# flupkede/codesearch

Hardware: AMD Instinct MI355X
Metric: chunks embedded+searched/sec over 10M×384 corpus; recall@10 vs CPU ref (higher is better)
Workload: dtype f32

## Files before the change

codesearch_amd/csrc/attention_split.hip:

```cpp
#include <cstdlib>
#include "encoder.hpp"
#include "split_f16.hpp"
#include "attention_shx_body.hpp"

#ifndef AT_STAMP
#define AT_STAMP(i)
#endif

namespace cs {

#ifndef CS_ATTN_PIPE_WAVES
#define CS_ATTN_PIPE_WAVES 3
#endif

constexpr int kAttnPipeDefault32 = 2, kAttnPipeDefault64 = 3;

#ifdef CS_DIAGNOSTICS
__global__ void __launch_bounds__(256, 2)
attention_sh2_kernel(const _Float16* __restrict__ qkvs, const int32_t* __restrict__ mask,
                     _Float16* __restrict__ ctxs, uint32_t* __restrict__ flag, uint32_t L, uint32_t H,
                     float scale_log2e) {
    extern __shared__ __attribute__((aligned(16))) char smem[];
    const uint32_t Lp = (L + 31) & ~31u;
    char* Kt = smem;
    char* Vt = Kt + (size_t)Lp * 128;
    float* madd = reinterpret_cast<float*>(Vt + (size_t)Lp * 128);
    int* last_valid_p = reinterpret_cast<int*>(madd + Lp);
    const int tid = threadIdx.x, lane = tid & 63;
    const int wave = __builtin_amdgcn_readfirstlane(tid >> 6);
    const int l31 = lane & 31, h = lane >> 5;
    const uint32_t head = blockIdx.x, b = blockIdx.y;
    const uint32_t nh = H / 32, nch = 3 * nh;
    const _Float16* base = qkvs + (size_t)b * L * nch * 64;
    bool ovf = false;

    AT_STAMP(0);
    if (tid == 0) *last_valid_p = 0;
    for (uint32_t ii = wave; ii < Lp / 8; ii += 4) {
        const uint32_t row = ii * 8 + (lane >> 3);
        const uint32_t key = row < L ? row : L - 1;
        const uint32_t ck = (lane & 7) ^ ((row >> 1) & 7);
        const uint32_t cv = (lane & 7) ^ (4 * ((row >> 1) & 1));
        sh_glds16(base + ((size_t)key * nch + nh + head) * 64 + ck * 8, Kt + ii * 1024);
        sh_glds16(base + ((size_t)key * nch + 2 * nh + head) * 64 + cv * 8, Vt + ii * 1024);
    }
    __syncthreads();
    for (uint32_t key = tid; key < Lp; key += 256) {
        const bool ok = key < L && mask[(size_t)b * L + key] != 0;
// ... 93 lines not shown
                oxx = __builtin_amdgcn_mfma_f32_32x32x16_f16(vh.v, pl[s].v, oxx, 0, 0, 0);
                oxx = __builtin_amdgcn_mfma_f32_32x32x16_f16(vl.v, ph[s].v, oxx, 0, 0, 0);
            }
        }
        lsum += __shfl_xor(lsum, 32, 64);
        const float inv = 1.0f / lsum;
        if (query < L) {
            _Float16* op = ctxs + (((size_t)b * L + query) * nh + head) * 64 + 4 * h;
#pragma unroll
            for (int g = 0; g < 4; ++g) {
                f16x4 hi, lo;
#pragma unroll
                for (int e = 0; e < 4; ++e) {
                    _Float16 a, bb;
                    ovf |= sh_split(fmaf(oxx[4 * g + e], kShLoInv, ohh[4 * g + e]) * inv, a, bb);
                    hi[e] = a; lo[e] = bb;
                }
                *reinterpret_cast<f16x4*>(op + 8 * g) = hi;
                *reinterpret_cast<f16x4*>(op + 32 + 8 * g) = lo;
            }
        }
    }
    AT_STAMP(2);
    if (ovf && flag) atomicOr(flag, 1u);
}
#endif

template <int NC, int POS = 0, int PIPE = 0>
__global__ void __launch_bounds__(256, NC == 1 ? (PIPE == 1 ? CS_ATTN_PIPE_WAVES : (PIPE >= 2 ? 4 : 2)) : 2)
attention_shx_kernel(const _Float16* __restrict__ qkvs, const int32_t* __restrict__ mask,
                     _Float16* __restrict__ ctxs, uint32_t* __restrict__ flag, uint32_t L, uint32_t H,
                     float scale_log2e, uint32_t HB, float* __restrict__ range_out,
                     const uint32_t* __restrict__ seq_unit, const uint32_t* __restrict__ unit_len,
                     const float* __restrict__ alibi_log2, uint32_t window) {
    extern __shared__ __attribute__((aligned(16))) char smem[];
    const AttnMemPlain mem;
    attention_shx_body<NC, AttnMemPlain, AttnMemPlain, POS, PIPE>(smem, mem, mem, qkvs, mask, ctxs, flag, L, H, scale_log2e, HB, range_out,
                                                            seq_unit, unit_len, blockIdx.x, blockIdx.y, blockIdx.z, gridDim.x,
                                                            gridDim.z, alibi_log2, window);
}

namespace {

struct ShxArgs {
    const _Float16* qkv; const int32_t* mask; _Float16* ctx; uint32_t* flag; uint32_t L, H; float scale_log2e; uint32_t hb;
    float* range_out; const uint32_t* seq_unit; const uint32_t* unit_len; const float* alibi_log2; uint32_t window;
};

template <int NC, int POS, int PIPE>
int32_t launch_shx_one(dim3 grid, size_t lds, hipStream_t s, const ShxArgs& a) {
    if (lds > 64 * 1024 - 256) {
        static PerDeviceOnce attr;
        CS_TRY(attr.run([&]() -> int32_t {
            CS_HIP(hipFuncSetAttribute(reinterpret_cast<const void*>(attention_shx_kernel<NC, POS, PIPE>),
                                       hipFuncAttributeMaxDynamicSharedMemorySize, 160 * 1024 - 64));
            return CS_OK;
        }));
    }
    hipLaunchKernelGGL((attention_shx_kernel<NC, POS, PIPE>), grid, dim3(256), lds, s, a.qkv, a.mask, a.ctx, a.flag, a.L, a.H,
                       a.scale_log2e, a.hb, a.range_out, a.seq_unit, a.unit_len, a.alibi_log2, a.window);
    CS_HIP(hipGetLastError());
    return CS_OK;
}

template <int NC>
int32_t launch_shx(int pos, int pipe, dim3 grid, size_t lds, hipStream_t s, const ShxArgs& a) {
#ifndef CS_DIAGNOSTICS
    constexpr int P = NC == 1 ? kAttnPipeDefault32 : kAttnPipeDefault64;
    (void)pipe;
    if (pos == 1) return launch_shx_one<NC, 1, P>(grid, lds, s, a);
    if (pos == 2) return launch_shx_one<NC, 2, P>(grid, lds, s, a);
    return launch_shx_one<NC, 0, P>(grid, lds, s, a);
#else
    if (pipe == 3) {
        if (pos == 1) return launch_shx_one<NC, 1, 3>(grid, lds, s, a);
        if (pos == 2) return launch_shx_one<NC, 2, 3>(grid, lds, s, a);
        return launch_shx_one<NC, 0, 3>(grid, lds, s, a);
    }
    if (pipe == 2) {
        if (pos == 1) return launch_shx_one<NC, 1, 2>(grid, lds, s, a);
        if (pos == 2) return launch_shx_one<NC, 2, 2>(grid, lds, s, a);
        return launch_shx_one<NC, 0, 2>(grid, lds, s, a);
    }
    if (pipe == 1) {
        if (pos == 1) return launch_shx_one<NC, 1, 1>(grid, lds, s, a);
        if (pos == 2) return launch_shx_one<NC, 2, 1>(grid, lds, s, a);
        return launch_shx_one<NC, 0, 1>(grid, lds, s, a);
    }
    if (pos == 1) return launch_shx_one<NC, 1, 0>(grid, lds, s, a);
    if (pos == 2) return launch_shx_one<NC, 2, 0>(grid, lds, s, a);
    return launch_shx_one<NC, 0, 0>(grid, lds, s, a);
#endif
}

}

int32_t launch_attention_sh2(const _Float16* qkv_split, const int32_t* mask, void* ctx_split, uint32_t* flag,
                             uint32_t B, uint32_t L, uint32_t H, uint32_t heads, hipStream_t s, float* range_out,
                             uint32_t* range_pairs, const uint32_t* seq_unit, const uint32_t* unit_len, const float* alibi,
                             uint32_t window) {
    if (alibi && window) return fail(CS_ERR_BAD_ARG, "attention: ALiBi and a local window together are not built");
    const float* alibi_log2 = alibi ? alibi + heads : nullptr;
    const int pos = alibi_log2 ? 1 : (window ? 2 : 0);
    if (range_pairs) *range_pairs = 0;
    const uint32_t dh = heads ? H / heads : 0;
    if ((dh != 32 && dh != 64) || H % heads)
        return fail(CS_ERR_UNSUPPORTED, "head_dim %u not supported (32 or 64)", dh);
    const size_t Lp = (L + 31) & ~31u;
    static const int pipe_env = [] { const char* e = cs_lab_env("CS_ATTN_PIPE"); return e && e[0] >= '0' && e[0] <= '3' ? e[0] - '0' : -1; }();
    ShxArgs a{qkv_split, mask, static_cast<_Float16*>(ctx_split), flag, L, H, 0.0f, 1u, range_out, seq_unit, unit_len, alibi_log2, window};
    if (dh == 64) {
        const size_t lds = 2 * 2 * 128 * 128 + Lp * sizeof(float) + 16;
        a.scale_log2e = (1.0f / sqrtf(64.0f)) * kLog2e;
        const int pipe = pipe_env < 0 ? kAttnPipeDefault64 : pipe_env;
        CS_TRY(launch_shx<2>(pos, pipe, dim3(heads, B, (L + 127) / 128), lds, s, a));
        if (range_pairs) *range_pairs = heads * B * ((L + 127) / 128) * 4;
        return CS_OK;
    }
    static const bool shx1 = [] { const char* e = cs_lab_env("CS_ATTN_SHX1"); return !(e && e[0] == '0'); }();
    if (shx1 || pos) {
        static const size_t lds_pad = [] { const char* e = cs_lab_env("CS_ATTN_LDS_PAD"); return e ? (size_t)std::atol(e) : (size_t)0; }();
        const size_t lds1 = 2 * 1 * 128 * 128 + Lp * sizeof(float) + 16 + lds_pad;
        static const bool pack_heads = [] { const char* e = cs_lab_env("CS_ATTN_PACK_HEADS"); return !(e && e[0] == '0'); }();
        uint32_t hb = !pack_heads ? 1u : (Lp <= 32 ? 4u : (Lp <= 64 ? 2u : 1u));
        while (heads % hb) hb >>= 1;
        a.scale_log2e = (1.0f / sqrtf(32.0f)) * kLog2e;
        a.hb = hb;
        const int pipe = pipe_env < 0 ? kAttnPipeDefault32 : pipe_env;
        CS_TRY(launch_shx<1>(pos, pipe, dim3(heads / hb, B, (L + 127) / 128), lds1, s, a));
        if (range_pairs) *range_pairs = (heads / hb) * B * ((L + 127) / 128) * 4;
        return CS_OK;
    }
#ifndef CS_DIAGNOSTICS
    return fail(CS_ERR_UNSUPPORTED, "attention: no kernel for head_dim %u", dh);
#else
    const size_t lds = 2 * Lp * 128 + Lp * sizeof(float) + 16;
    if (lds > 160 * 1024 - 64) return fail(CS_ERR_UNSUPPORTED, "sequence length %u exceeds the LDS-resident K/V limit", L);
    static PerDeviceOnce attr_set;
    CS_TRY(attr_set.run([&]() -> int32_t {
        CS_HIP(hipFuncSetAttribute(reinterpret_cast<const void*>(attention_sh2_kernel),
                                   hipFuncAttributeMaxDynamicSharedMemorySize, 160 * 1024 - 64));
        return CS_OK;
// ... 10 lines not shown
```

codesearch_amd/csrc/attention_shx_body.hpp:

```cpp
#pragma once

#include "encoder.hpp"
#include "split_f16.hpp"

#ifndef AT_STAMP
#define AT_STAMP(i)
#endif
#ifndef CS_ATTN_ARITH
#define CS_ATTN_ARITH 2
#endif
#ifndef CS_ATTN_LAZY_RESCALE
#define CS_ATTN_LAZY_RESCALE 4.0f
#endif
#ifndef CS_ATTN_PIPE_FENCE
#define CS_ATTN_PIPE_FENCE __builtin_amdgcn_sched_barrier(0)
#endif

namespace cs {

typedef __fp16 h16x2 __attribute__((ext_vector_type(2)));

constexpr float kLog2e = 1.4426950408889634f;
constexpr float kMaskedLog2 = -3.0e38f;

union Frag8 {
    f16x8 v;
    uint32_t u[4];
    uint2 d[2];
};

typedef short s16x4 __attribute__((ext_vector_type(4)));

union FragTr {
    f16x8 v;
    s16x4 q[2];
};

__device__ __forceinline__ void split_pair_rtz_ng(float a, float b, uint32_t& hi, uint32_t& lo) {
    const h16x2 h = __builtin_amdgcn_cvt_pkrtz(a, b);
    const h16x2 l = __builtin_amdgcn_cvt_pkrtz((a - (float)h[0]) * kShLoScale, (b - (float)h[1]) * kShLoScale);
    hi = __builtin_bit_cast(uint32_t, h);
    lo = __builtin_bit_cast(uint32_t, l);
}

__device__ __forceinline__ float mix_residual_lo(float e, uint32_t hpair) {
    float r;
    asm("v_fma_mix_f32 %0, %1, -1.0, %2 op_sel_hi:[1,0,0]" : "=v"(r) : "v"(hpair), "v"(e));
    return r;
}
__device__ __forceinline__ float mix_residual_hi(float e, uint32_t hpair) {
    float r;
    asm("v_fma_mix_f32 %0, %1, -1.0, %2 op_sel:[1,0,0] op_sel_hi:[1,0,0]" : "=v"(r) : "v"(hpair), "v"(e));
    return r;
}

__device__ __forceinline__ float xhalf_max_swap(float t) {
    const uint32_t u = __builtin_bit_cast(uint32_t, t);
    const auto r = __builtin_amdgcn_permlane32_swap(u, u, false, false);
    const uint32_t a = r[0], b = r[1];
    return fmaxf(__builtin_bit_cast(float, a), __builtin_bit_cast(float, b));
}

struct AttnMemPlain {
    __device__ __forceinline__ f16x8 ld16(const _Float16* p) const { return *reinterpret_cast<const f16x8*>(p); }
    __device__ __forceinline__ f16x8 stage_load(const _Float16* src, char* lds_piece) const { sh_glds16(src, lds_piece); return f16x8{}; }
    __device__ __forceinline__ void stage_store(char*, int, f16x8) const {}
    __device__ __forceinline__ void st8(_Float16* p, f16x4 v) const { *reinterpret_cast<f16x4*>(p) = v; }
};

template <int NC, class MQ, class MO, int POS = 0, int PIPE = 0>
__device__ __forceinline__ void
attention_shx_body(char* smem, const MQ& mq, const MO& mo, const _Float16* qkvs, const int32_t* __restrict__ mask,
                   _Float16* ctxs, uint32_t* __restrict__ flag, uint32_t L, uint32_t H,
                   float scale_log2e, uint32_t HB, float* __restrict__ range_out,
                   const uint32_t* __restrict__ seq_unit, const uint32_t* __restrict__ unit_len,
                   uint32_t bx, uint32_t by, uint32_t bz, uint32_t gx, uint32_t gz, const float* __restrict__ alibi_log2 = nullptr,
                   uint32_t window = 0) {
    constexpr bool ALIBI = POS == 1, WINDOW = POS == 2;
    constexpr bool IMM = PIPE >= 2;
    constexpr bool EARLY = PIPE == 3;
    const float wlimit = (float)window;
    constexpr int KT = 128;
    const uint32_t Lp = (L + 31) & ~31u;
    char* Kt = smem;
    char* Vt = Kt + (size_t)NC * KT * 128;
    float* madd = reinterpret_cast<float*>(Vt + (size_t)NC * KT * 128);
    int* last_valid_p = reinterpret_cast<int*>(madd + Lp);
    const int tid = threadIdx.x, lane = tid & 63;
    const int wave = __builtin_amdgcn_readfirstlane(tid >> 6);
    const int l31 = lane & 31, h = lane >> 5;
    const uint32_t wq = 4 / HB, hsub = (uint32_t)wave / wq, qt = (uint32_t)wave % wq;
    const uint32_t head = bx * HB + hsub, b = by, qb = bz;
    Kt += (size_t)hsub * (KT / HB) * 128;
    Vt += (size_t)hsub * (KT / HB) * 128;
    const uint32_t nh = H / (32 * NC), nch = 3 * nh * NC;
    const _Float16* base = qkvs + (size_t)b * L * nch * 64;
    bool ovf = false;

    AT_STAMP(0);
    if (tid == 0) *last_valid_p = 0;

    const int kswz = (l31 >> 1) & 7;
    int k_hi[2], k_lo[2];
#pragma unroll
    for (int s = 0; s < 2; ++s) {
        k_hi[s] = ((2 * s + h) ^ kswz) * 16;
        k_lo[s] = ((4 + 2 * s + h) ^ kswz) * 16;
    }
    const int vq = (lane & 15) >> 2, vp = lane & 3, vg = (lane >> 4) & 1;
    const int vfv = 4 * ((vq >> 1) & 1);
    const int v_hi = (4 * h + vq) * 128 + (((2 * vg + (vp >> 1)) ^ vfv) * 16) + 8 * (vp & 1);
    const int v_lo = v_hi ^ 64;

    const bool wave_live = qb * 128 + qt * 32 < L;
    const uint32_t query = qb * 128 + qt * 32 + l31;
    const uint32_t qsrc = query < L ? query : L - 1;
    float neg_slope = 0.0f;
    const float qpos = (float)query - (float)(4 * h);
    if constexpr (ALIBI) neg_slope = -alibi_log2[head];
    f16x8 qh[NC][2], ql[NC][2];
#pragma unroll
    for (int c = 0; c < NC; ++c) {
        const _Float16* qp = base + ((size_t)qsrc * nch + head * NC + c) * 64 + 8 * h;
#pragma unroll
        for (int s = 0; s < 2; ++s) {
            qh[c][s] = mq.ld16(qp + 16 * s);
            ql[c][s] = mq.ld16(qp + 32 + 16 * s);
        }
    }
#if CS_ATTN_ARITH == 2 && !defined(CS_ATTN_SCALAR_SOFTMAX)
    f16x8 qhs[NC][2];
#pragma unroll
    for (int c = 0; c < NC; ++c)
#pragma unroll
        for (int s = 0; s < 2; ++s) {
            qhs[c][s] = qh[c][s] * (_Float16)kShLoInv;
            ql[c][s] = ql[c][s] * (_Float16)kShLoInv;
        }
#endif
    sh_f32x16 ohh[NC], oxx[NC];
#pragma unroll
    for (int c = 0; c < NC; ++c)
#pragma unroll
        for (int r = 0; r < 16; ++r) { ohh[c][r] = 0.0f; oxx[c][r] = 0.0f; }
    float m = -__builtin_huge_valf(), lsum = 0.0f;

    auto stage = [&](uint32_t st) {
        const uint32_t live = Lp - st * KT < (uint32_t)KT ? Lp - st * KT : (uint32_t)KT;
        for (uint32_t i0 = qt; i0 < live / 8; i0 += 4 * wq) {
            f16x8 rk[4][NC], rv[4][NC];
#pragma unroll
            for (int u = 0; u < 4; ++u) {
                const uint32_t ii = i0 + u * wq;
                if (ii < live / 8) {
                    const uint32_t row = ii * 8 + (lane >> 3);
                    const uint32_t gk = st * KT + row;
                    const uint32_t key = gk < L ? gk : L - 1;
                    const uint32_t ck = (lane & 7) ^ ((row >> 1) & 7);
                    const uint32_t cv = (lane & 7) ^ (4 * ((row >> 1) & 1));
#pragma unroll
                    for (int c = 0; c < NC; ++c) {
                        rk[u][c] = mq.stage_load(base + ((size_t)key * nch + (nh + head) * NC + c) * 64 + ck * 8, Kt + (size_t)c * KT * 128 + ii * 1024);
                        rv[u][c] = mq.stage_load(base + ((size_t)key * nch + (2 * nh + head) * NC + c) * 64 + cv * 8, Vt + (size_t)c * KT * 128 + ii * 1024);
                    }
                }
            }
#pragma unroll
            for (int u = 0; u < 4; ++u) {
                const uint32_t ii = i0 + u * wq;
                if (ii < live / 8) {
#pragma unroll
                    for (int c = 0; c < NC; ++c) {
                        mq.stage_store(Kt + (size_t)c * KT * 128 + ii * 1024, lane, rk[u][c]);
                        mq.stage_store(Vt + (size_t)c * KT * 128 + ii * 1024, lane, rv[u][c]);
                    }
                }
            }
        }
    };
    stage(0);
    __syncthreads();
    for (uint32_t key = tid; key < Lp; key += 256) {
        const bool ok = key < L && mask[(size_t)b * L + key] != 0;
        madd[key] = ok ? 0.0f : kMaskedLog2;
        if (ok) atomicMax(last_valid_p, (int)key);
    }
    asm volatile("s_waitcnt vmcnt(0)" ::: "memory");
    __syncthreads();
    const uint32_t ntiles = (uint32_t)(*last_valid_p) / 32 + 1;

    typedef __attribute__((address_space(3))) char* lds_char_p;
    typedef __attribute__((address_space(3))) const f16x8* lds_f16x8_cp;
    typedef __attribute__((address_space(3))) const sh_f32x4* lds_f32x4_cp;
    uint32_t ka[4] = {0, 0, 0, 0}, va[2] = {0, 0}, ma0 = 0;
    if constexpr (IMM) {
        const uint32_t k0 = (uint32_t)(uintptr_t)(lds_char_p)Kt + (uint32_t)l31 * 128u, v0 = (uint32_t)(uintptr_t)(lds_char_p)Vt;
#pragma unroll
        for (int s = 0; s < 2; ++s) { ka[s] = k0 + (uint32_t)k_hi[s]; ka[2 + s] = k0 + (uint32_t)k_lo[s]; }
        va[0] = v0 + (uint32_t)v_hi;
        va[1] = v0 + (uint32_t)v_lo;
        ma0 = (uint32_t)(uintptr_t)(lds_char_p)reinterpret_cast<char*>(madd) + 16u * (uint32_t)h;
#pragma unroll
        for (int i = 0; i < 4; ++i) asm volatile("" : "+v"(ka[i]));
        asm volatile("" : "+v"(va[0]), "+v"(va[1]), "+v"(ma0));
    }

    for (uint32_t st = 0; st * 4 < ntiles; ++st) {
        if constexpr (WINDOW) {
            if (st * KT > qb * 128 + 127 + window || st * KT + (KT - 1) + window < qb * 128) continue;
        }
        if (st > 0) {
            __syncthreads();
            stage(st);
            asm volatile("s_waitcnt vmcnt(0)" ::: "memory");
            __syncthreads();
        }
        if (!wave_live) continue;
        const uint32_t kt_end = ntiles - st * 4 < 4 ? ntiles - st * 4 : 4;
        const uint32_t ma_st = ma0 + st * 512u;
        uint32_t kl_lo = 0, kl_hi = kt_end;
        if constexpr (WINDOW) {
            const int q0 = (int)(qb * 128 + qt * 32), w = (int)window, t0 = (int)(st * 4);
            const int first = q0 - 31 - w > 0 ? (q0 - 31 - w + 31) / 32 : 0, past = (q0 + 31 + w) / 32 + 1;
            kl_lo = (uint32_t)(first > t0 ? first - t0 : 0);
            kl_hi = past - t0 < (int)kt_end ? (uint32_t)(past - t0 > 0 ? past - t0 : 0) : kt_end;
        }
        auto compute_s = [&](uint32_t kl, sh_f32x16& hh, sh_f32x16& xx) __attribute__((always_inline)) {
#pragma unroll
            for (int r = 0; r < 16; ++r) { hh[r] = 0.0f; xx[r] = 0.0f; }
            if constexpr (EARLY) {
                f16x8 kf[NC][4];
#pragma unroll
                for (int c = 0; c < NC; ++c)
#pragma unroll
                    for (int i = 0; i < 4; ++i) kf[c][i] = *(lds_f16x8_cp)(uintptr_t)(ka[i] + (uint32_t)(c * KT * 128) + kl * 4096u);
                __builtin_amdgcn_sched_barrier(0);
#pragma unroll
                for (int c = 0; c < NC; ++c)
#pragma unroll
                    for (int s = 0; s < 2; ++s) {
                        hh = __builtin_amdgcn_mfma_f32_32x32x16_f16(kf[c][s], qh[c][s], hh, 0, 0, 0);
#if CS_ATTN_ARITH == 2 && !defined(CS_ATTN_SCALAR_SOFTMAX)
                        hh = __builtin_amdgcn_mfma_f32_32x32x16_f16(kf[c][s], ql[c][s], hh, 0, 0, 0);
                        hh = __builtin_amdgcn_mfma_f32_32x32x16_f16(kf[c][2 + s], qhs[c][s], hh, 0, 0, 0);
#else
                        xx = __builtin_amdgcn_mfma_f32_32x32x16_f16(kf[c][s], ql[c][s], xx, 0, 0, 0);
                        xx = __builtin_amdgcn_mfma_f32_32x32x16_f16(kf[c][2 + s], qh[c][s], xx, 0, 0, 0);
#endif
                    }
                return;
            }
#pragma unroll
            for (int c = 0; c < NC; ++c) {
                const char* kr = Kt + (size_t)c * KT * 128 + (size_t)(kl * 32 + l31) * 128;
#pragma unroll
                for (int s = 0; s < 2; ++s) {
                    f16x8 kh, kl8;
                    if constexpr (IMM) {
                        kh = *(lds_f16x8_cp)(uintptr_t)(ka[s] + (uint32_t)(c * KT * 128) + kl * 4096u);
                        kl8 = *(lds_f16x8_cp)(uintptr_t)(ka[2 + s] + (uint32_t)(c * KT * 128) + kl * 4096u);
                    } else {
                        kh = *reinterpret_cast<const f16x8*>(kr + k_hi[s]);
                        kl8 = *reinterpret_cast<const f16x8*>(kr + k_lo[s]);
                    }
                    hh = __builtin_amdgcn_mfma_f32_32x32x16_f16(kh, qh[c][s], hh, 0, 0, 0);
#if CS_ATTN_ARITH == 2 && !defined(CS_ATTN_SCALAR_SOFTMAX)
                    hh = __builtin_amdgcn_mfma_f32_32x32x16_f16(kh, ql[c][s], hh, 0, 0, 0);
                    hh = __builtin_amdgcn_mfma_f32_32x32x16_f16(kl8, qhs[c][s], hh, 0, 0, 0);
#else
                    xx = __builtin_amdgcn_mfma_f32_32x32x16_f16(kh, ql[c][s], xx, 0, 0, 0);
                    xx = __builtin_amdgcn_mfma_f32_32x32x16_f16(kl8, qh[c][s], xx, 0, 0, 0);
#endif
                }
            }
        };
        auto finish_tile = [&](uint32_t kl, sh_f32x16& hh, sh_f32x16& xx) __attribute__((always_inline)) {
            const uint32_t kt = st * 4 + kl;
#ifndef CS_ATTN_SCALAR_SOFTMAX
            sh_f32x2 p2[8];
            float tmax = -__builtin_huge_valf();
            const sh_f32x2 lo_inv2 = {kShLoInv, kShLoInv}, scale2 = {scale_log2e, scale_log2e};
#pragma unroll
            for (int g = 0; g < 4; ++g) {
                sh_f32x4 ma;
                if constexpr (IMM) ma = *(lds_f32x4_cp)(uintptr_t)(ma_st + (kl * 32u + 8u * g) * 4u);
                else ma = *reinterpret_cast<const sh_f32x4*>(madd + kt * 32 + 8 * g + 4 * h);
#pragma unroll
                for (int e2 = 0; e2 < 2; ++e2) {
                    const int r = 4 * g + 2 * e2;
                    const sh_f32x2 x2 = {xx[r], xx[r + 1]}, h2 = {hh[r], hh[r + 1]};
                    sh_f32x2 m2 = {ma[2 * e2], ma[2 * e2 + 1]};
                    if constexpr (ALIBI) {
                        const float d0 = qpos - (float)(kt * 32 + 8 * g + 2 * e2);
                        m2[0] = fmaf(neg_slope, fabsf(d0), m2[0]);
                        m2[1] = fmaf(neg_slope, fabsf(d0 - 1.0f), m2[1]);
                    }
                    if constexpr (WINDOW) {
                        const float d0 = qpos - (float)(kt * 32 + 8 * g + 2 * e2);
                        m2[0] = fabsf(d0) > wlimit ? kMaskedLog2 : m2[0];
                        m2[1] = fabsf(d0 - 1.0f) > wlimit ? kMaskedLog2 : m2[1];
                    }
#if CS_ATTN_ARITH == 2
                    (void)x2; (void)lo_inv2;
                    const sh_f32x2 s2 = __builtin_elementwise_fma(h2, scale2, m2);
#else
                    const sh_f32x2 s2 = __builtin_elementwise_fma(__builtin_elementwise_fma(x2, lo_inv2, h2), scale2, m2);
#endif
                    p2[r / 2] = s2;
                    tmax = fmaxf(tmax, fmaxf(s2[0], s2[1]));
                }
            }
            if constexpr (IMM) tmax = xhalf_max_swap(tmax);
            else tmax = fmaxf(tmax, __shfl_xor(tmax, 32, 64));
#if CS_ATTN_ARITH == 2
            if (__any(tmax > m + CS_ATTN_LAZY_RESCALE)) {
#else
            if (__any(tmax > m)) {
#endif
                const float mnew = fmaxf(m, tmax);
                const float alpha = __builtin_amdgcn_exp2f(m - mnew);
                lsum *= alpha;
#pragma unroll
                for (int c = 0; c < NC; ++c)
#pragma unroll
                    for (int r = 0; r < 16; ++r) { ohh[c][r] *= alpha; oxx[c][r] *= alpha; }
                m = mnew;
            }
            typedef __attribute__((address_space(3))) s16x4* lds_s16x4_p;
            FragTr vhe[NC][2], vle[NC][2];
            if constexpr (EARLY) {
#pragma unroll
                for (int c = 0; c < NC; ++c)
#pragma unroll
                    for (int s = 0; s < 2; ++s) {
                        const uint32_t off = (uint32_t)(c * KT * 128) + kl * 4096u + (uint32_t)(s * 16 * 128);
                        vhe[c][s].q[0] = __builtin_amdgcn_ds_read_tr16_b64_v4i16((lds_s16x4_p)(uintptr_t)(va[0] + off));
                        vhe[c][s].q[1] = __builtin_amdgcn_ds_read_tr16_b64_v4i16((lds_s16x4_p)(uintptr_t)(va[0] + off + 1024u));
                        vle[c][s].q[0] = __builtin_amdgcn_ds_read_tr16_b64_v4i16((lds_s16x4_p)(uintptr_t)(va[1] + off));
                        vle[c][s].q[1] = __builtin_amdgcn_ds_read_tr16_b64_v4i16((lds_s16x4_p)(uintptr_t)(va[1] + off + 1024u));
                    }
                __builtin_amdgcn_sched_barrier(0);
            }
#if CS_ATTN_ARITH == 2
            const sh_f32x2 m2v = {m - 11.0f, m - 11.0f};
#else
            const sh_f32x2 m2v = {m, m};
#endif
            sh_f32x2 ps2 = {0.0f, 0.0f};
            Frag8 ph[2], pl[2];
            const sh_f32x2 lo_scale2 = {kShLoScale, kShLoScale};
#pragma unroll
            for (int i = 0; i < 8; ++i) {
                const sh_f32x2 d2 = p2[i] - m2v;
                const sh_f32x2 e2 = {__builtin_amdgcn_exp2f(d2[0]), __builtin_amdgcn_exp2f(d2[1])};
                ps2 += e2;
                const h16x2 hi = __builtin_amdgcn_cvt_pkrtz(e2[0], e2[1]);
#if CS_ATTN_ARITH == 2
                (void)lo_scale2;
                const uint32_t hib = __builtin_bit_cast(uint32_t, hi);
                const h16x2 lo = __builtin_amdgcn_cvt_pkrtz(mix_residual_lo(e2[0], hib), mix_residual_hi(e2[1], hib));
#else
                const sh_f32x2 back = {(float)hi[0], (float)hi[1]};
                const sh_f32x2 r2 = (e2 - back) * lo_scale2;
                const h16x2 lo = __builtin_amdgcn_cvt_pkrtz(r2[0], r2[1]);
#endif
                ph[i >> 2].u[i & 3] = __builtin_bit_cast(uint32_t, hi);
                pl[i >> 2].u[i & 3] = __builtin_bit_cast(uint32_t, lo);
            }
            lsum += ps2[0] + ps2[1];
#else
            float tmax = -__builtin_huge_valf();
#pragma unroll
            for (int g = 0; g < 4; ++g) {
                const sh_f32x4 ma = *reinterpret_cast<const sh_f32x4*>(madd + kt * 32 + 8 * g + 4 * h);
#pragma unroll
                for (int e = 0; e < 4; ++e) {
                    const int r = 4 * g + e;
                    float me = ma[e];
                    if constexpr (ALIBI) me = fmaf(neg_slope, fabsf(qpos - (float)(kt * 32 + 8 * g + e)), me);
                    if constexpr (WINDOW) me = fabsf(qpos - (float)(kt * 32 + 8 * g + e)) > wlimit ? kMaskedLog2 : me;
                    hh[r] = fmaf(fmaf(xx[r], kShLoInv, hh[r]), scale_log2e, me);
                    tmax = fmaxf(tmax, hh[r]);
                }
            }
            tmax = fmaxf(tmax, __shfl_xor(tmax, 32, 64));
            if (__any(tmax > m)) {
                const float mnew = fmaxf(m, tmax);
                const float alpha = __builtin_amdgcn_exp2f(m - mnew);
                lsum *= alpha;
#pragma unroll
                for (int c = 0; c < NC; ++c)
#pragma unroll
                    for (int r = 0; r < 16; ++r) { ohh[c][r] *= alpha; oxx[c][r] *= alpha; }
                m = mnew;
            }
            float psum = 0.0f;
#pragma unroll
            for (int r = 0; r < 16; ++r) {
                hh[r] = __builtin_amdgcn_exp2f(hh[r] - m);
                psum += hh[r];
            }
            lsum += psum;
            Frag8 ph[2], pl[2];
#pragma unroll
            for (int s = 0; s < 2; ++s)
#pragma unroll
                for (int w2 = 0; w2 < 4; ++w2) {
#ifdef CS_ATTN_P_HI_ONLY
                    const f16x2 pr = __builtin_convertvector(sh_f32x2{hh[8 * s + 2 * w2], hh[8 * s + 2 * w2 + 1]}, f16x2);
                    ph[s].u[w2] = __builtin_bit_cast(uint32_t, pr);
                    pl[s].u[w2] = 0u;
#else
                    split_pair_rtz_ng(hh[8 * s + 2 * w2], hh[8 * s + 2 * w2 + 1], ph[s].u[w2], pl[s].u[w2]);
#endif
                }
#endif
#ifdef CS_ATTN_SCALAR_SOFTMAX
            typedef __attribute__((address_space(3))) s16x4* lds_s16x4_p;
            FragTr vhe[NC][2], vle[NC][2];
#endif
#pragma unroll
            for (int c = 0; c < NC; ++c) {
                const char* vr = Vt + (size_t)c * KT * 128 + (size_t)kl * 32 * 128;
#pragma unroll
                for (int s = 0; s < 2; ++s) {
                    FragTr vh, vl;
                    if constexpr (EARLY) {
                        vh = vhe[c][s];
                        vl = vle[c][s];
                    } else if constexpr (IMM) {
                        const uint32_t off = (uint32_t)(c * KT * 128) + kl * 4096u + (uint32_t)(s * 16 * 128);
                        vh.q[0] = __builtin_amdgcn_ds_read_tr16_b64_v4i16((lds_s16x4_p)(uintptr_t)(va[0] + off));
                        vh.q[1] = __builtin_amdgcn_ds_read_tr16_b64_v4i16((lds_s16x4_p)(uintptr_t)(va[0] + off + 1024u));
                        vl.q[0] = __builtin_amdgcn_ds_read_tr16_b64_v4i16((lds_s16x4_p)(uintptr_t)(va[1] + off));
                        vl.q[1] = __builtin_amdgcn_ds_read_tr16_b64_v4i16((lds_s16x4_p)(uintptr_t)(va[1] + off + 1024u));
                    } else {
                    vh.q[0] = __builtin_amdgcn_ds_read_tr16_b64_v4i16((lds_s16x4_p)(vr + s * 16 * 128 + v_hi));
                    vh.q[1] = __builtin_amdgcn_ds_read_tr16_b64_v4i16((lds_s16x4_p)(vr + s * 16 * 128 + 8 * 128 + v_hi));
                    vl.q[0] = __builtin_amdgcn_ds_read_tr16_b64_v4i16((lds_s16x4_p)(vr + s * 16 * 128 + v_lo));
                    vl.q[1] = __builtin_amdgcn_ds_read_tr16_b64_v4i16((lds_s16x4_p)(vr + s * 16 * 128 + 8 * 128 + v_lo));
                    }
                    ohh[c] = __builtin_amdgcn_mfma_f32_32x32x16_f16(vh.v, ph[s].v, ohh[c], 0, 0, 0);
#if CS_ATTN_ARITH == 2 && !defined(CS_ATTN_SCALAR_SOFTMAX)
                    ohh[c] = __builtin_amdgcn_mfma_f32_32x32x16_f16(vh.v, pl[s].v, ohh[c], 0, 0, 0);
#elif !defined(CS_ATTN_P_HI_ONLY)
                    oxx[c] = __builtin_amdgcn_mfma_f32_32x32x16_f16(vh.v, pl[s].v, oxx[c], 0, 0, 0);
#endif
                    oxx[c] = __builtin_amdgcn_mfma_f32_32x32x16_f16(vl.v, ph[s].v, oxx[c], 0, 0, 0);
                }
            }
        };
        if constexpr (PIPE == 0) {
            for (uint32_t kl = kl_lo; kl < kl_hi; ++kl) {
                sh_f32x16 hh, xx;
                compute_s(kl, hh, xx);
                finish_tile(kl, hh, xx);
            }
        } else if constexpr (IMM) {
#pragma unroll
            for (uint32_t kl = 0; kl < 4; ++kl) {
                if (kl >= kl_lo && kl < kl_hi) {
                    sh_f32x16 hh, xx;
                    compute_s(kl, hh, xx);
                    finish_tile(kl, hh, xx);
                }
            }
        } else {
            sh_f32x16 hhA, xxA, hhB, xxB;
            if (kl_lo < kl_hi) compute_s(kl_lo, hhA, xxA);
            for (uint32_t kl = kl_lo; kl < kl_hi; kl += 2) {
                if (kl + 1 < kl_hi) compute_s(kl + 1, hhB, xxB);
                CS_ATTN_PIPE_FENCE;
                finish_tile(kl, hhA, xxA);
                if (kl + 1 < kl_hi) {
                    if (kl + 2 < kl_hi) compute_s(kl + 2, hhA, xxA);
                    CS_ATTN_PIPE_FENCE;
                    finish_tile(kl + 1, hhB, xxB);
                }
            }
        }
    }
    lsum += __shfl_xor(lsum, 32, 64);
    const float inv = lsum > 0.0f ? 1.0f / lsum : 0.0f;
    float rlo = 0.0f, rhi = 0.0f;
    if (wave_live && query < L) {
#pragma unroll
        for (int c = 0; c < NC; ++c) {
            _Float16* op = ctxs + (((size_t)b * L + query) * nh + head) * NC * 64 + c * 64 + 4 * h;
#pragma unroll
            for (int g = 0; g < 4; ++g) {
                f16x4 hi, lo;
#pragma unroll
                for (int e = 0; e < 4; ++e) {
                    _Float16 a, bb;
                    const float o = fmaf(oxx[c][4 * g + e], kShLoInv, ohh[c][4 * g + e]) * inv;
                    ovf |= sh_split(o, a, bb);
                    hi[e] = a; lo[e] = bb;
                    rlo = fminf(rlo, o);
                    rhi = fmaxf(rhi, o);
                }
                mo.st8(op + 8 * g, hi);
                mo.st8(op + 32 + 8 * g, lo);
            }
        }
    }
    AT_STAMP(2);
    if (ovf && flag) atomicOr(flag, 1u);
    if (range_out) {
        if (unit_len && query >= unit_len[seq_unit[b]]) rlo = rhi = 0.0f;
#pragma unroll
        for (int o = 32; o > 0; o >>= 1) {
            rlo = fminf(rlo, __shfl_xor(rlo, o, 64));
            rhi = fmaxf(rhi, __shfl_xor(rhi, o, 64));
        }
        if (lane == 0) {
            const size_t blk = ((size_t)by * gz + bz) * gx + bx;
            _Float16 a, bb;
            (void)sh_split(rlo, a, bb);
            range_out[(blk * 4 + wave) * 2] = fmaf((float)bb, kShLoInv, (float)a);
            (void)sh_split(rhi, a, bb);
            range_out[(blk * 4 + wave) * 2 + 1] = fmaf((float)bb, kShLoInv, (float)a);
        }
    }
}

}
```

codesearch_amd/csrc/small_forward.hip:

```cpp
#include "small_forward.hpp"

#include "attention_shx_body.hpp"
#include "encoder_rows.hpp"
#include "gemm_epilogue.hpp"
#include "split_f16.hpp"

#include <type_traits>

namespace cs {

namespace {

typedef unsigned int sf_u32x4 __attribute__((ext_vector_type(4)));
typedef unsigned int sf_u32x2 __attribute__((ext_vector_type(2)));

constexpr int SF_GRID = 96;
constexpr int SF_W_BYTES = 16 * 12 * 128;
constexpr int SF_AROW = 384 * 4 + 16;
constexpr int SF_AIMG = 16 * SF_AROW;
constexpr int SF_RED = 4 * 16 * 17 * 4;
constexpr int SF_ATT = 2 * 128 * 128 + 512 * 4 + 16;
constexpr int SF_OFF_AIMG = SF_W_BYTES, SF_OFF_RED = SF_W_BYTES + SF_AIMG, SF_OFF_ATT = SF_W_BYTES;
constexpr int SF_LDS = SF_W_BYTES + (SF_ATT > SF_AIMG + SF_RED ? SF_ATT : SF_AIMG + SF_RED);
constexpr int SC1 = 16;
// ... 238 lines not shown
    using E_RESID = std::integral_constant<int, SH_OUT_F32_RESID>;
    using E_PART = std::integral_constant<int, SH_OUT_PARTIAL>;

    constexpr uint32_t NT_QKV = 3 * H / 16, NT_H = H / 16, NT_I = I / 16;
    const float scale_log2e = (1.0f / sqrtf(32.0f)) * kLog2e;

    {
        const SfMap m(NT_QKV, blk);
        if (m.active) sf_w_prefetch(lds_w, a.layers[0].wqkv, m.nt, KC_H, 0, KC_H, wave, lane);
        asm volatile("s_waitcnt vmcnt(0)" ::: "memory");
        __syncthreads();
    }

    for (uint32_t l = 0; l < a.n_layers; ++l) {
        const SfLayer ly = a.layers[l];
        {
            const SfMap m(NT_QKV, blk);
            if (m.active) {
                const float* gw = l ? a.layers[l - 1].ln2_g : a.emb_g;
                const float* bw = l ? a.layers[l - 1].ln2_b : a.emb_b;
                const float* pb = l ? a.layers[l - 1].bdown : nullptr;
                for (uint32_t mt = m.mt0; mt < MT; mt += m.mt_step) {
                    ln_prologue(mt, gw, bw, l ? 1 : 2, pb, m.nt == 0, a.XA, bXA);
                    tile(E_SPLIT{}, true, nullptr, nullptr, 0, 0, mt, m.nt, ly.bqkv, &bQ, 3 * H, nullptr, a.QKVS, 0);
                }
            }
        }
        if (!barrier(ly.wo, NT_H, KC_H, 5 * l + 1)) return;
        {
            const uint32_t hgroups = a.heads / a.hb, qblocks = (a.L + 127) / 128;
            const uint32_t tasks = hgroups * a.B * qblocks;
            for (uint32_t t = blk; t < tasks; t += SF_GRID) {
                const uint32_t bx = t % hgroups, by = (t / hgroups) % a.B, bz = t / (hgroups * a.B);
                attention_shx_body<1>(lds + SF_OFF_ATT, bQ, bC, a.QKVS, a.mask, a.CTXS, a.flag, a.L, H, scale_log2e, a.hb, nullptr,
                                      nullptr, nullptr, bx, by, bz, hgroups, qblocks);
                __syncthreads();
            }
        }
        if (!barrier(nullptr, 0, 0, 5 * l + 2)) return;
        {
            const SfMap m(NT_H, blk);
            if (m.active)
                for (uint32_t mt = m.mt0; mt < MT; mt += m.mt_step)
                    tile(E_RESID{}, false, &bC, a.CTXS, KC_H, 0, mt, m.nt, ly.bo, &bY, H, a.Y, nullptr, 0);
        }
        if (!barrier(ly.wup, NT_I, KC_H, 5 * l + 3)) return;
        {
            const SfMap m(NT_I, blk);
            if (m.active)
                for (uint32_t mt = m.mt0; mt < MT; mt += m.mt_step) {
                    ln_prologue(mt, ly.ln1_g, ly.ln1_b, 0, nullptr, m.nt == 0, a.X, bX);
                    tile(E_GELU{}, true, nullptr, nullptr, 0, 0, mt, m.nt, ly.bup, &bM, I, nullptr, a.MIDS, 0);
                }
        }
        if (!barrier(ly.wdown, NT_H, KC_I, 5 * l + 4, true)) return;
        {
            const SfMap m(NT_H, blk);
            if (m.active)
                for (uint32_t mt = 0; mt < MT; ++mt)
                    tile(E_PART{}, false, &bM, a.MIDS, KC_I, m.mt0 * (KC_I / 4), mt, m.nt, nullptr, &bP, H, a.PARTS, nullptr, m.mt0);
        }
        const bool last = l + 1 == a.n_layers;
        if (!barrier(last ? nullptr : a.layers[l + 1].wqkv, NT_QKV, KC_H, 5 * l + 5)) return;
    }
    {
        const SfLayer ly = a.layers[a.n_layers - 1];
        for (uint32_t t = 4 * blk + wave; t < T; t += 4 * SF_GRID) {
// ... 45 lines not shown
```

Baseline: 4.625 billion.

## Remap attention blocks to a 1D grid so each XCD keeps one head group

Launches the attention kernel on a flattened 1D grid and remaps the linear block id so that all query blocks of a (batch, head) group land on the same XCD, assuming round-robin block dispatch across the eight XCDs. The goal is to keep a group's K/V reads inside one XCD's L2 instead of spreading them across all of them. This adds index arithmetic per block plus a check on the total block count, and the old grid order remains available only as a diagnostic fallback.

Result: no change. 4.621 billion (-0.1%).

```diff
diff --git a/codesearch_amd/csrc/attention_split.hip b/codesearch_amd/csrc/attention_split.hip
--- a/codesearch_amd/csrc/attention_split.hip
+++ b/codesearch_amd/csrc/attention_split.hip
@@ -2,6 +2,7 @@
 #include "encoder.hpp"
 #include "split_f16.hpp"
 #include "attention_shx_body.hpp"
+#include "attn_dispatch.hpp"
 
 #ifndef AT_STAMP
 #define AT_STAMP(i)
@@ -173,12 +174,20 @@
                      _Float16* __restrict__ ctxs, uint32_t* __restrict__ flag, uint32_t L, uint32_t H,
                      float scale_log2e, uint32_t HB, float* __restrict__ range_out,
                      const uint32_t* __restrict__ seq_unit, const uint32_t* __restrict__ unit_len,
-                     const float* __restrict__ alibi_log2, uint32_t window) {
+                     const float* __restrict__ alibi_log2, uint32_t window, uint32_t gx, uint32_t groups, uint32_t gz,
+                     uint32_t grid_order) {
     extern __shared__ __attribute__((aligned(16))) char smem[];
     const AttnMemPlain mem;
+    AttnBlock blk = attn_dispatch(blockIdx.x, groups, gz);
+#ifdef CS_DIAGNOSTICS
+    if (grid_order) blk = attn_dispatch_grid_order(blockIdx.x, groups);
+#else
+    (void)grid_order;
+#endif
+    const uint32_t group = __builtin_amdgcn_readfirstlane(blk.group), bz = __builtin_amdgcn_readfirstlane(blk.qb);
+    const uint32_t by = __builtin_amdgcn_readfirstlane(group / gx), bx = group - by * gx;
     attention_shx_body<NC, AttnMemPlain, AttnMemPlain, POS, PIPE>(smem, mem, mem, qkvs, mask, ctxs, flag, L, H, scale_log2e, HB, range_out,
-                                                            seq_unit, unit_len, blockIdx.x, blockIdx.y, blockIdx.z, gridDim.x,
-                                                            gridDim.z, alibi_log2, window);
+                                                            seq_unit, unit_len, bx, by, bz, gx, gz, alibi_log2, window);
 }
 
 namespace {
@@ -198,8 +207,13 @@
             return CS_OK;
         }));
     }
-    hipLaunchKernelGGL((attention_shx_kernel<NC, POS, PIPE>), grid, dim3(256), lds, s, a.qkv, a.mask, a.ctx, a.flag, a.L, a.H,
-                       a.scale_log2e, a.hb, a.range_out, a.seq_unit, a.unit_len, a.alibi_log2, a.window);
+    const uint64_t groups = (uint64_t)grid.x * grid.y, blocks = groups * grid.z;
+    if (blocks > 0x7fffffffull) return fail(CS_ERR_UNSUPPORTED, "attention: %llu blocks exceed the grid limit", (unsigned long long)blocks);
+    const char* de = cs_lab_env("CS_ATTN_DISPATCH");
+    const uint32_t grid_order = de && de[0] == '0';
+    hipLaunchKernelGGL((attention_shx_kernel<NC, POS, PIPE>), dim3((uint32_t)blocks), dim3(256), lds, s, a.qkv, a.mask, a.ctx, a.flag,
+                       a.L, a.H, a.scale_log2e, a.hb, a.range_out, a.seq_unit, a.unit_len, a.alibi_log2, a.window, grid.x,
+                       (uint32_t)groups, grid.z, grid_order);
     CS_HIP(hipGetLastError());
     return CS_OK;
 }
diff --git a/codesearch_amd/csrc/attn_dispatch.hpp b/codesearch_amd/csrc/attn_dispatch.hpp
--- /dev/null
+++ b/codesearch_amd/csrc/attn_dispatch.hpp
@@ -0,0 +1,32 @@
+#pragma once
+
+#include <cstdint>
+
+#if defined(__HIPCC__) || defined(__CUDACC__)
+#define CS_ATTN_DISPATCH_FN __host__ __device__ inline
+#else
+#define CS_ATTN_DISPATCH_FN inline
+#endif
+
+namespace cs {
+
+struct AttnBlock {
+    uint32_t group;
+    uint32_t qb;
+};
+
+CS_ATTN_DISPATCH_FN AttnBlock attn_dispatch(uint32_t lin, uint32_t groups, uint32_t QB) {
+    const uint32_t whole = groups & ~7u;
+    if (lin < whole * QB) {
+        const uint32_t xcd = lin & 7u, slot = lin >> 3;
+        return AttnBlock{(slot / QB) * 8u + xcd, slot % QB};
+    }
+    const uint32_t rest = lin - whole * QB, tail = groups - whole;
+    return AttnBlock{whole + rest % tail, rest / tail};
+}
+
+CS_ATTN_DISPATCH_FN AttnBlock attn_dispatch_grid_order(uint32_t lin, uint32_t groups) {
+    return AttnBlock{lin % groups, lin / groups};
+}
+
+}
```

## Fold PV low-part into single accumulator, add paired 64-key attention step

Applied to the files above, without the earlier changes.

Scales the high P fragment by the low-part inverse so the V-low product accumulates into the main output accumulator. This drops the second set of 16-float accumulators per chunk by default and frees registers. It also adds an opt-in PIPE=4 path that computes two 32-key score tiles together and rescales once per pair. The mask pass now uses per-wave ballots instead of LDS atomicMax. The fused small_forward kernel instantiates the default pipe (2) explicitly. Folding the scaled term into one f32 accumulator may slightly change rounding.

After: 4.633 billion before, 4.633 billion after (median of 2 runs). No clear change (+0.0%).

```diff
diff --git a/codesearch_amd/csrc/attention_shx_body.hpp b/codesearch_amd/csrc/attention_shx_body.hpp
--- a/codesearch_amd/csrc/attention_shx_body.hpp
+++ b/codesearch_amd/csrc/attention_shx_body.hpp
@@ -1,6 +1,7 @@
 #pragma once
 
 #include "encoder.hpp"
+#include <type_traits>
 #include "split_f16.hpp"
 
 #ifndef AT_STAMP
@@ -12,6 +13,14 @@
 #ifndef CS_ATTN_LAZY_RESCALE
 #define CS_ATTN_LAZY_RESCALE 4.0f
 #endif
+#if CS_ATTN_ARITH == 2 && !defined(CS_ATTN_SCALAR_SOFTMAX)
+#define CS_ATTN_ONE_ACC 1
+#else
+#define CS_ATTN_ONE_ACC 0
+#endif
+#ifndef CS_ATTN_PV_ACC
+#define CS_ATTN_PV_ACC 1
+#endif
 #ifndef CS_ATTN_PIPE_FENCE
 #define CS_ATTN_PIPE_FENCE __builtin_amdgcn_sched_barrier(0)
 #endif
@@ -20,8 +29,15 @@
 
 typedef __fp16 h16x2 __attribute__((ext_vector_type(2)));
 
+#ifndef CS_ATTN_PIPE_DEFAULT32
+#define CS_ATTN_PIPE_DEFAULT32 2
+#endif
+constexpr int kAttnPipeDefault32 = CS_ATTN_PIPE_DEFAULT32, kAttnPipeDefault64 = 3;
+
 constexpr float kLog2e = 1.4426950408889634f;
 constexpr float kMaskedLog2 = -3.0e38f;
+
+__device__ __forceinline__ float attn_mask_add(bool valid) { return valid ? 0.0f : kMaskedLog2; }
 
 union Frag8 {
     f16x8 v;
@@ -79,13 +95,15 @@
     constexpr bool ALIBI = POS == 1, WINDOW = POS == 2;
     constexpr bool IMM = PIPE >= 2;
     constexpr bool EARLY = PIPE == 3;
+    constexpr bool PAIR = PIPE == 4;
+    static_assert(!PAIR || CS_ATTN_ONE_ACC, "the 64-key step is written for the one-accumulator arithmetic");
     const float wlimit = (float)window;
     constexpr int KT = 128;
     const uint32_t Lp = (L + 31) & ~31u;
     char* Kt = smem;
     char* Vt = Kt + (size_t)NC * KT * 128;
     float* madd = reinterpret_cast<float*>(Vt + (size_t)NC * KT * 128);
-    int* last_valid_p = reinterpret_cast<int*>(madd + Lp);
+    int* last_valid_w = reinterpret_cast<int*>(madd + Lp);
     const int tid = threadIdx.x, lane = tid & 63;
     const int wave = __builtin_amdgcn_readfirstlane(tid >> 6);
     const int l31 = lane & 31, h = lane >> 5;
@@ -98,7 +116,6 @@
     bool ovf = false;
 
     AT_STAMP(0);
-    if (tid == 0) *last_valid_p = 0;
 
     const int kswz = (l31 >> 1) & 7;
     int k_hi[2], k_lo[2];
@@ -128,7 +145,7 @@
             ql[c][s] = mq.ld16(qp + 32 + 16 * s);
         }
     }
-#if CS_ATTN_ARITH == 2 && !defined(CS_ATTN_SCALAR_SOFTMAX)
+#if CS_ATTN_ONE_ACC
     f16x8 qhs[NC][2];
 #pragma unroll
     for (int c = 0; c < NC; ++c)
@@ -138,11 +155,17 @@
             ql[c][s] = ql[c][s] * (_Float16)kShLoInv;
         }
 #endif
-    sh_f32x16 ohh[NC], oxx[NC];
+    constexpr bool PV_ONE = CS_ATTN_ONE_ACC && (PIPE == 4 || CS_ATTN_PV_ACC == 1);
+    constexpr int NX = PV_ONE ? 0 : NC;
+    sh_f32x16 ohh[NC], oxx[NX ? NX : 1];
 #pragma unroll
     for (int c = 0; c < NC; ++c)
 #pragma unroll
-        for (int r = 0; r < 16; ++r) { ohh[c][r] = 0.0f; oxx[c][r] = 0.0f; }
+        for (int r = 0; r < 16; ++r) ohh[c][r] = 0.0f;
+#pragma unroll
+    for (int c = 0; c < NX; ++c)
+#pragma unroll
+        for (int r = 0; r < 16; ++r) oxx[c][r] = 0.0f;
     float m = -__builtin_huge_valf(), lsum = 0.0f;
 
     auto stage = [&](uint32_t st) {
@@ -179,15 +202,24 @@
         }
     };
     stage(0);
-    __syncthreads();
-    for (uint32_t key = tid; key < Lp; key += 256) {
-        const bool ok = key < L && mask[(size_t)b * L + key] != 0;
-        madd[key] = ok ? 0.0f : kMaskedLog2;
-        if (ok) atomicMax(last_valid_p, (int)key);
+    int wlast = 0;
+    for (uint32_t key0 = tid; key0 < Lp; key0 += 512) {
+        const uint32_t key1 = key0 + 256;
+        const int32_t mv0 = key0 < L ? mask[(size_t)b * L + key0] : 0;
+        const int32_t mv1 = key1 < L ? mask[(size_t)b * L + key1] : 0;
+        madd[key0] = attn_mask_add(mv0 != 0);
+        if (key1 < Lp) madd[key1] = attn_mask_add(mv1 != 0);
+        const uint64_t b0 = __ballot(mv0 != 0), b1 = __ballot(mv1 != 0);
+        if (b0) wlast = (int)(key0 - lane) + 63 - __builtin_clzll(b0);
+        if (b1) wlast = (int)(key1 - lane) + 63 - __builtin_clzll(b1);
     }
+    if (lane == 0) last_valid_w[wave] = wlast;
     asm volatile("s_waitcnt vmcnt(0)" ::: "memory");
     __syncthreads();
-    const uint32_t ntiles = (uint32_t)(*last_valid_p) / 32 + 1;
+    const int lv01 = last_valid_w[0] > last_valid_w[1] ? last_valid_w[0] : last_valid_w[1];
+    const int lv23 = last_valid_w[2] > last_valid_w[3] ? last_valid_w[2] : last_valid_w[3];
+    const int last_valid = __builtin_amdgcn_readfirstlane(lv01 > lv23 ? lv01 : lv23);
+    const uint32_t ntiles = (uint32_t)last_valid / 32 + 1;
 
     typedef __attribute__((address_space(3))) char* lds_char_p;
     typedef __attribute__((address_space(3))) const f16x8* lds_f16x8_cp;
@@ -240,7 +272,7 @@
 #pragma unroll
                     for (int s = 0; s < 2; ++s) {
                         hh = __builtin_amdgcn_mfma_f32_32x32x16_f16(kf[c][s], qh[c][s], hh, 0, 0, 0);
-#if CS_ATTN_ARITH == 2 && !defined(CS_ATTN_SCALAR_SOFTMAX)
+#if CS_ATTN_ONE_ACC
                         hh = __builtin_amdgcn_mfma_f32_32x32x16_f16(kf[c][s], ql[c][s], hh, 0, 0, 0);
                         hh = __builtin_amdgcn_mfma_f32_32x32x16_f16(kf[c][2 + s], qhs[c][s], hh, 0, 0, 0);
 #else
@@ -264,7 +296,7 @@
                         kl8 = *reinterpret_cast<const f16x8*>(kr + k_lo[s]);
                     }
                     hh = __builtin_amdgcn_mfma_f32_32x32x16_f16(kh, qh[c][s], hh, 0, 0, 0);
-#if CS_ATTN_ARITH == 2 && !defined(CS_ATTN_SCALAR_SOFTMAX)
+#if CS_ATTN_ONE_ACC
                     hh = __builtin_amdgcn_mfma_f32_32x32x16_f16(kh, ql[c][s], hh, 0, 0, 0);
                     hh = __builtin_amdgcn_mfma_f32_32x32x16_f16(kl8, qhs[c][s], hh, 0, 0, 0);
 #else
@@ -274,11 +306,55 @@
                 }
             }
         };
-        auto finish_tile = [&](uint32_t kl, sh_f32x16& hh, sh_f32x16& xx) __attribute__((always_inline)) {
+        auto compute_s2 = [&](uint32_t kl, sh_f32x16& a, sh_f32x16& b) __attribute__((always_inline)) {
+#if CS_ATTN_ONE_ACC
+#pragma unroll
+            for (int r = 0; r < 16; ++r) { a[r] = 0.0f; b[r] = 0.0f; }
+#pragma unroll
+            for (int c = 0; c < NC; ++c)
+#pragma unroll
+                for (int s = 0; s < 2; ++s) {
+                    const uint32_t off = (uint32_t)(c * KT * 128) + kl * 4096u;
+                    const f16x8 kha = *(lds_f16x8_cp)(uintptr_t)(ka[s] + off), khb = *(lds_f16x8_cp)(uintptr_t)(ka[s] + off + 4096u);
+                    const f16x8 kla = *(lds_f16x8_cp)(uintptr_t)(ka[2 + s] + off), klb = *(lds_f16x8_cp)(uintptr_t)(ka[2 + s] + off + 4096u);
+                    a = __builtin_amdgcn_mfma_f32_32x32x16_f16(kha, qh[c][s], a, 0, 0, 0);
+                    b = __builtin_amdgcn_mfma_f32_32x32x16_f16(khb, qh[c][s], b, 0, 0, 0);
+                    a = __builtin_amdgcn_mfma_f32_32x32x16_f16(kha, ql[c][s], a, 0, 0, 0);
+                    b = __builtin_amdgcn_mfma_f32_32x32x16_f16(khb, ql[c][s], b, 0, 0, 0);
+                    a = __builtin_amdgcn_mfma_f32_32x32x16_f16(kla, qhs[c][s], a, 0, 0, 0);
+                    b = __builtin_amdgcn_mfma_f32_32x32x16_f16(klb, qhs[c][s], b, 0, 0, 0);
+                }
+#else
+            (void)kl; (void)a; (void)b;
+#endif
+        };
+#if CS_ATTN_ARITH == 2
+        constexpr float kLag = CS_ATTN_LAZY_RESCALE;
+#else
+        constexpr float kLag = 0.0f;
+#endif
+        auto move_reference = [&](float tmax) __attribute__((always_inline)) {
+            if (__any(tmax > m + kLag)) {
+                const float mnew = fmaxf(m, tmax);
+                const float alpha = __builtin_amdgcn_exp2f(m - mnew);
+                lsum *= alpha;
+#pragma unroll
+                for (int c = 0; c < NC; ++c)
+#pragma unroll
+                    for (int r = 0; r < 16; ++r) {
+                        ohh[c][r] *= alpha;
+                        if constexpr (NX > 0) oxx[c][r] *= alpha;
+                    }
+                m = mnew;
+            }
+        };
+        auto tile_phase = [&](uint32_t kl, sh_f32x16& hh, sh_f32x16& xx, sh_f32x2 (&p2)[8], float& tmax_io, auto phase) __attribute__((always_inline)) {
+            constexpr int PH = decltype(phase)::value;
             const uint32_t kt = st * 4 + kl;
 #ifndef CS_ATTN_SCALAR_SOFTMAX
-            sh_f32x2 p2[8];
-            float tmax = -__builtin_huge_valf();
+            float& tmax = tmax_io;
+            if constexpr (PH != 2) {
+            tmax = -__builtin_huge_valf();
             const sh_f32x2 lo_inv2 = {kShLoInv, kShLoInv}, scale2 = {scale_log2e, scale_log2e};
 #pragma unroll
             for (int g = 0; g < 4; ++g) {
@@ -310,21 +386,12 @@
                     tmax = fmaxf(tmax, fmaxf(s2[0], s2[1]));
                 }
             }
-            if constexpr (IMM) tmax = xhalf_max_swap(tmax);
-            else tmax = fmaxf(tmax, __shfl_xor(tmax, 32, 64));
-#if CS_ATTN_ARITH == 2
-            if (__any(tmax > m + CS_ATTN_LAZY_RESCALE)) {
-#else
-            if (__any(tmax > m)) {
-#endif
-                const float mnew = fmaxf(m, tmax);
-                const float alpha = __builtin_amdgcn_exp2f(m - mnew);
-                lsum *= alpha;
-#pragma unroll
-                for (int c = 0; c < NC; ++c)
-#pragma unroll
-                    for (int r = 0; r < 16; ++r) { ohh[c][r] *= alpha; oxx[c][r] *= alpha; }
-                m = mnew;
+            }
+            if constexpr (PH == 1) return;
+            if constexpr (PH == 0) {
+                if constexpr (IMM) tmax = xhalf_max_swap(tmax);
+                else tmax = fmaxf(tmax, __shfl_xor(tmax, 32, 64));
+                move_reference(tmax);
             }
             typedef __attribute__((address_space(3))) s16x4* lds_s16x4_p;
             FragTr vhe[NC][2], vle[NC][2];
@@ -368,7 +435,15 @@
                 pl[i >> 2].u[i & 3] = __builtin_bit_cast(uint32_t, lo);
             }
             lsum += ps2[0] + ps2[1];
-#else
+#if CS_ATTN_ONE_ACC
+            Frag8 phs[2];
+            if constexpr (PV_ONE) {
+#pragma unroll
+                for (int s = 0; s < 2; ++s) phs[s].v = ph[s].v * (_Float16)kShLoInv;
+            }
+#endif
+#else
+            (void)p2; (void)PH;
             float tmax = -__builtin_huge_valf();
 #pragma unroll
             for (int g = 0; g < 4; ++g) {
@@ -391,7 +466,10 @@
 #pragma unroll
                 for (int c = 0; c < NC; ++c)
 #pragma unroll
-                    for (int r = 0; r < 16; ++r) { ohh[c][r] *= alpha; oxx[c][r] *= alpha; }
+                    for (int r = 0; r < 16; ++r) {
+                        ohh[c][r] *= alpha;
+                        if constexpr (NX > 0) oxx[c][r] *= alpha;
+                    }
                 m = mnew;
             }
             float psum = 0.0f;
@@ -441,16 +519,49 @@
                     vl.q[1] = __builtin_amdgcn_ds_read_tr16_b64_v4i16((lds_s16x4_p)(vr + s * 16 * 128 + 8 * 128 + v_lo));
                     }
                     ohh[c] = __builtin_amdgcn_mfma_f32_32x32x16_f16(vh.v, ph[s].v, ohh[c], 0, 0, 0);
-#if CS_ATTN_ARITH == 2 && !defined(CS_ATTN_SCALAR_SOFTMAX)
+#if CS_ATTN_ONE_ACC
                     ohh[c] = __builtin_amdgcn_mfma_f32_32x32x16_f16(vh.v, pl[s].v, ohh[c], 0, 0, 0);
-#elif !defined(CS_ATTN_P_HI_ONLY)
+                    if constexpr (PV_ONE) ohh[c] = __builtin_amdgcn_mfma_f32_32x32x16_f16(vl.v, phs[s].v, ohh[c], 0, 0, 0);
+                    else oxx[c] = __builtin_amdgcn_mfma_f32_32x32x16_f16(vl.v, ph[s].v, oxx[c], 0, 0, 0);
+#else
+#if !defined(CS_ATTN_P_HI_ONLY)
                     oxx[c] = __builtin_amdgcn_mfma_f32_32x32x16_f16(vh.v, pl[s].v, oxx[c], 0, 0, 0);
 #endif
                     oxx[c] = __builtin_amdgcn_mfma_f32_32x32x16_f16(vl.v, ph[s].v, oxx[c], 0, 0, 0);
+#endif
                 }
             }
         };
-        if constexpr (PIPE == 0) {
+        auto finish_tile = [&](uint32_t kl, sh_f32x16& hh, sh_f32x16& xx) __attribute__((always_inline)) {
+            sh_f32x2 p2[8];
+            float tmax;
+            tile_phase(kl, hh, xx, p2, tmax, std::integral_constant<int, 0>{});
+        };
+        if constexpr (PAIR) {
+#pragma unroll
+            for (uint32_t kp = 0; kp < 4; kp += 2) {
+                const bool la = kp >= kl_lo && kp < kl_hi, lb = kp + 1 >= kl_lo && kp + 1 < kl_hi;
+                if (la && lb) {
+                    sh_f32x16 hhA, hhB;
+                    compute_s2(kp, hhA, hhB);
+                    sh_f32x2 pA[8], pB[8];
+                    float tA, tB;
+                    tile_phase(kp, hhA, hhA, pA, tA, std::integral_constant<int, 1>{});
+                    tile_phase(kp + 1, hhB, hhB, pB, tB, std::integral_constant<int, 1>{});
+                    move_reference(xhalf_max_swap(fmaxf(tA, tB)));
+                    tile_phase(kp, hhA, hhA, pA, tA, std::integral_constant<int, 2>{});
+                    tile_phase(kp + 1, hhB, hhB, pB, tB, std::integral_constant<int, 2>{});
+                } else if (la) {
+                    sh_f32x16 hh, xx;
+                    compute_s(kp, hh, xx);
+                    finish_tile(kp, hh, xx);
+                } else if (lb) {
+                    sh_f32x16 hh, xx;
+                    compute_s(kp + 1, hh, xx);
+                    finish_tile(kp + 1, hh, xx);
+                }
+            }
+        } else if constexpr (PIPE == 0) {
             for (uint32_t kl = kl_lo; kl < kl_hi; ++kl) {
                 sh_f32x16 hh, xx;
                 compute_s(kl, hh, xx);
@@ -493,7 +604,9 @@
 #pragma unroll
                 for (int e = 0; e < 4; ++e) {
                     _Float16 a, bb;
-                    const float o = fmaf(oxx[c][4 * g + e], kShLoInv, ohh[c][4 * g + e]) * inv;
+                    float o = ohh[c][4 * g + e];
+                    if constexpr (NX > 0) o = fmaf(oxx[c][4 * g + e], kShLoInv, o);
+                    o *= inv;
                     ovf |= sh_split(o, a, bb);
                     hi[e] = a; lo[e] = bb;
                     rlo = fminf(rlo, o);
diff --git a/codesearch_amd/csrc/attention_split.hip b/codesearch_amd/csrc/attention_split.hip
--- a/codesearch_amd/csrc/attention_split.hip
+++ b/codesearch_amd/csrc/attention_split.hip
@@ -13,7 +13,6 @@
 #define CS_ATTN_PIPE_WAVES 3
 #endif
 
-constexpr int kAttnPipeDefault32 = 2, kAttnPipeDefault64 = 3;
 
 #ifdef CS_DIAGNOSTICS
 __global__ void __launch_bounds__(256, 2)
@@ -213,6 +212,11 @@
     if (pos == 2) return launch_shx_one<NC, 2, P>(grid, lds, s, a);
     return launch_shx_one<NC, 0, P>(grid, lds, s, a);
 #else
+    if (pipe == 4) {
+        if (pos == 1) return launch_shx_one<NC, 1, 4>(grid, lds, s, a);
+        if (pos == 2) return launch_shx_one<NC, 2, 4>(grid, lds, s, a);
+        return launch_shx_one<NC, 0, 4>(grid, lds, s, a);
+    }
     if (pipe == 3) {
         if (pos == 1) return launch_shx_one<NC, 1, 3>(grid, lds, s, a);
         if (pos == 2) return launch_shx_one<NC, 2, 3>(grid, lds, s, a);
@@ -248,7 +252,8 @@
     if ((dh != 32 && dh != 64) || H % heads)
         return fail(CS_ERR_UNSUPPORTED, "head_dim %u not supported (32 or 64)", dh);
     const size_t Lp = (L + 31) & ~31u;
-    static const int pipe_env = [] { const char* e = cs_lab_env("CS_ATTN_PIPE"); return e && e[0] >= '0' && e[0] <= '3' ? e[0] - '0' : -1; }();
+    const char* pipe_e = cs_lab_env("CS_ATTN_PIPE");
+    const int pipe_env = pipe_e && pipe_e[0] >= '0' && pipe_e[0] <= '4' ? pipe_e[0] - '0' : -1;
     ShxArgs a{qkv_split, mask, static_cast<_Float16*>(ctx_split), flag, L, H, 0.0f, 1u, range_out, seq_unit, unit_len, alibi_log2, window};
     if (dh == 64) {
         const size_t lds = 2 * 2 * 128 * 128 + Lp * sizeof(float) + 16;
diff --git a/codesearch_amd/csrc/small_forward.hip b/codesearch_amd/csrc/small_forward.hip
--- a/codesearch_amd/csrc/small_forward.hip
+++ b/codesearch_amd/csrc/small_forward.hip
@@ -294,7 +294,7 @@
             const uint32_t tasks = hgroups * a.B * qblocks;
             for (uint32_t t = blk; t < tasks; t += SF_GRID) {
                 const uint32_t bx = t % hgroups, by = (t / hgroups) % a.B, bz = t / (hgroups * a.B);
-                attention_shx_body<1>(lds + SF_OFF_ATT, bQ, bC, a.QKVS, a.mask, a.CTXS, a.flag, a.L, H, scale_log2e, a.hb, nullptr,
+                attention_shx_body<1, Sc1Buf, Sc1Buf, 0, kAttnPipeDefault32>(lds + SF_OFF_ATT, bQ, bC, a.QKVS, a.mask, a.CTXS, a.flag, a.L, H, scale_log2e, a.hb, nullptr,
                                       nullptr, nullptr, bx, by, bz, hgroups, qblocks);
                 __syncthreads();
             }
```
